# ivario123/r7020e-visual-odometry

Hardware: AMD Instinct MI355X
Metric: stereo frames/sec @1242x375 (SIFT detect+describe x2 + stereo matchFeatures) (higher is better)
Workload: dtype f32 (i8 MFMA for exact descriptor dot products); 1 GPU; BASELINE configs[1]: SIFT detect+describe + BF match on 1242x375 synthetic stereo, ~2k keypoints/image; rows=375, cols=1242, parallelism=frames sharded over 1 GPU(s)

## Files before the change

### r7020e-visual-odometry_amd/csrc/sift.hip

```cpp
#include "vo_internal.h"
#include <cstdlib>
#include <cstring>
#include <cmath>
#include <algorithm>
#include <utility>
#include <type_traits>
#include <mutex>

namespace vo {

struct Kern { float k[VO_SIFT_MAX_RADIUS + 1]; int r; float* nb; int nb_pitch, nb_rows, nb_cols; };

static int desc_radius_cap(const Pyramid& py, const vo_sift_params& p);

void build_pyramid_geometry(Pyramid& py, int rows, int cols, int n_img, const vo_sift_params& p)
{
    memset(&py, 0, sizeof(py));
    const int L = p.n_octave_layers;
    py.L = L;
    py.n_img = n_img;
    py.n_oct = vo_num_octaves(rows, cols, p.upsample);
    int R = p.upsample ? rows * 2 : rows, C = p.upsample ? cols * 2 : cols;
    size_t off = 0;
    size_t tmp_plane = 0;
// ... 1839 lines not shown
#ifndef VO_CPL2_MAXC
#define VO_CPL2_MAXC 1400
#endif
#ifndef VO_BLUR_MAX_TH
#define VO_BLUR_MAX_TH 128
#endif
#ifndef VO_BLUR_WAVES
#define VO_BLUR_WAVES 2048
#endif
        constexpr int kMaxTH = VO_BLUR_MAX_TH, kWaveTarget = VO_BLUR_WAVES, kCpl2MaxC = VO_CPL2_MAXC;
        const bool base = name[7] == 'b';
        const int cpl = (!base && C <= kCpl2MaxC) ? 2 : 4;
        const int n_strips = (C + 64 * cpl - 1) / (64 * cpl);
        const long rows_total = (long)R * n_strips * grid.z;
        int TH = (int)std::min<long>(base ? std::min(kMaxTH, kBaseMaxTH) : kMaxTH, rows_total / kWaveTarget);
        TH = std::max(BS_P, TH / BS_P * BS_P);
        if (R >= TH && R > RAD + BS_P + 2) {
            const int n_bands = (R + TH - 1) / TH;
#define VO_BS_GO(T, CP)                                                                                        \
    do {                                                                                                       \
        const int ns_ = (C + bs_sw(RAD, CP, T) - 1) / bs_sw(RAD, CP, T);                                       \
        VO_LAUNCH_NAMED(name, (k_blur_stream<RAD, T, CP>), dim3(ns_ * n_bands * (int)grid.z), dim3(64), 0, s, src, plane, \
                        dplane, pitch, R, C, g, K, ns_, n_bands, TH, isrc, in_rows, in_cols);                     \
    } while (0)
            if (base && src == nullptr) VO_BS_GO(5, 4);
            else if (base) VO_BS_GO(1, 4);
            else if (cpl == 2) VO_BS_GO(0, 2);
            else VO_BS_GO(0, 4);
#undef VO_BS_GO
            return true;
        }
    }
    if (lds > 64 * 1024) raise_lds_limit((const void*)k_blur_fused<RAD, MODE>);
    VO_LAUNCH_NAMED(MODE == 0 ? "k_blur_fused" : "k_blur_base", (k_blur_fused<RAD, MODE>), grid, dim3(256), lds, s, src,
                    plane, dplane, pitch, R, C, g, d, K, isrc, in_rows, in_cols);
    return false;
}

template <int MODE>
static bool launch_blur(dim3 grid, hipStream_t s, const float* src, size_t plane, size_t dplane, int pitch, int R, int C, float* g,
                        float* d, const Kern& K, const ImageSrc& isrc, int in_rows, int in_cols,
                        const char* name = MODE == 0 ? "k_blur_fused" : "k_blur_base")
{
    switch (K.r) {
    case 5: return launch_blur_r<5, MODE>(grid, s, src, plane, dplane, pitch, R, C, g, d, K, isrc, in_rows, in_cols, name);
    case 6: return launch_blur_r<6, MODE>(grid, s, src, plane, dplane, pitch, R, C, g, d, K, isrc, in_rows, in_cols, name);
    case 8: return launch_blur_r<8, MODE>(grid, s, src, plane, dplane, pitch, R, C, g, d, K, isrc, in_rows, in_cols, name);
    case 10: return launch_blur_r<10, MODE>(grid, s, src, plane, dplane, pitch, R, C, g, d, K, isrc, in_rows, in_cols, name);
    case 13: return launch_blur_r<13, MODE>(grid, s, src, plane, dplane, pitch, R, C, g, d, K, isrc, in_rows, in_cols, name);
    default: return launch_blur_r<0, MODE>(grid, s, src, plane, dplane, pitch, R, C, g, d, K, isrc, in_rows, in_cols, name);
    }
}

static float ext_threshold(const Pyramid& py, const vo_sift_params& p)
{
    return (float)floor(0.5 * p.contrast_threshold / py.L * 255.0);
}

struct SmallPlan { int o_small, rtab, cap, bcap; size_t lds; };
static SmallPlan small_plan(const Pyramid& py)
{
    SmallPlan sp{py.n_oct, 0, 0, 0, 0};
    int maxr = 0;
    for (int i = 1; i < py.L + 3; ++i) maxr = std::max(maxr, py.krad[i]);
    for (int o = py.n_oct - 1; o >= 1; --o) {
        int rt = 0, ct = 0, cap = 0, bcap = 0;
        bool fits = true;
        for (int q = o; q < py.n_oct; ++q) {
            fits = fits && py.oct[q].rows * py.oct[q].cols <= VO_SMALL_PX;
            cap = std::max(cap, py.oct[q].rows * py.oct[q].cols);
            if (q > o) bcap = std::max(bcap, py.oct[q].rows * py.oct[q].cols);
            rt = std::max(rt, py.oct[q].rows + 2 * maxr);
            ct = std::max(ct, py.oct[q].cols + 2 * maxr);
        }
        cap = (cap + 3) & ~3;
        bcap = (bcap + 3) & ~3;
        const size_t lds = sizeof(float) * (3 * (size_t)cap + bcap) + sizeof(int) * (rt + ct);
        if (!fits || lds > 160 * 1024) break;
        sp = SmallPlan{o, rt, cap, bcap, lds};
    }
    return sp;
}

int sift_small_octave(const Pyramid& py) { return small_plan(py).o_small; }

void sift_enqueue_small(const Pyramid& py, SiftBuffers& b, int n_img, hipStream_t s, const Pyramid* d_py)
{
    const SmallPlan sp = small_plan(py);
    if (sp.o_small >= py.n_oct) return;

    raise_lds_limit((const void*)k_small_pyr);
    VO_LAUNCH_NAMED("k_blur_small", k_small_pyr, dim3(n_img), dim3(VO_SMALL_T), sp.lds, s, d_py, b.arena, sp.o_small,
                    sp.rtab, sp.cap, sp.bcap);
}

void sift_enqueue_pyramid(const Pyramid& py, SiftBuffers& b, const ImageSrc& src, int n_img, const vo_sift_params& p,
                          hipStream_t s, const Pyramid* d_py, hipEvent_t ev_o0)
{
    const int L = py.L;
    float* A = b.arena;
    const SmallPlan sp = small_plan(py);
    const int o_small = sp.o_small;
    bool base_done = false;
    for (int o = 0; o < py.n_oct; ++o) {
        const OctGeom& g = py.oct[o];
        const int R = g.rows, C = g.cols;
        if (o == o_small) break;
        dim3 gf((C + FT_W - 1) / FT_W, (R + FT_H - 1) / FT_H, n_img);
        if (o == 0) {
            Kern K0 = make_kern(py, 0);
            const int rows = p.upsample ? R / 2 : R, cols = p.upsample ? C / 2 : C;
            const int r0 = K0.r;
            const bool stream_r = r0 == 5 || r0 == 6 || r0 == 8 || r0 == 10 || r0 == 13;
            if (p.upsample && stream_r && R >= 64) {
                launch_blur<0>(gf, s, nullptr, 0, py.istride, g.pitch, R, C, A + g.g_off[0], nullptr, K0, src, rows, cols,
                               "k_blur_base");
            } else {
                const dim3 qg((g.pitch / 4 + 255) / 256, R, n_img);
                if (p.upsample)
                    VO_LAUNCH(k_base_src<true>, qg, dim3(256), 0, s, src, rows, cols, b.tmp, g.plane, g.pitch, R, C, n_img);
                else
                    VO_LAUNCH(k_base_src<false>, qg, dim3(256), 0, s, src, rows, cols, b.tmp, g.plane, g.pitch, R, C, n_img);
                launch_blur<0>(gf, s, b.tmp, g.plane, py.istride, g.pitch, R, C, A + g.g_off[0], nullptr, K0, src, 0, 0,
                               "k_blur_base");
            }
        } else if (!base_done) {
            const OctGeom& pg = py.oct[o - 1];
            VO_LAUNCH(k_down, dim3((C + 255) / 256, R, n_img), dim3(256), 0, s, A + pg.g_off[L], py.istride, pg.pitch,
                      A + g.g_off[0], py.istride, g.pitch, C);
        }
        base_done = false;
        for (int i = 1; i < L + 3; ++i) {
            Kern K = make_kern(py, i);
            const bool emit = i == L && o + 1 < o_small;
            if (emit) {
                const OctGeom& ng = py.oct[o + 1];
                K.nb = A + ng.g_off[0];
                K.nb_pitch = ng.pitch; K.nb_rows = ng.rows; K.nb_cols = ng.cols;
            }
            const bool streamed = launch_blur<0>(gf, s, A + g.g_off[i - 1], py.istride, py.istride, g.pitch, R, C,
                                                 A + g.g_off[i], nullptr, K, src, 0, 0);
            if (emit) base_done = streamed;
        }
        if (o == 0 && ev_o0) hipEventRecord(ev_o0, s);
    }
}

#ifndef VO_FEATURE_GRID
#define VO_FEATURE_GRID 32768
#endif
constexpr int kFeatureGrid = VO_FEATURE_GRID;

void sift_enqueue_extrema(const Pyramid& py, SiftBuffers& b, int n_img, const vo_sift_params& p, hipStream_t s,
                          const Pyramid* d_py, int o_begin, int o_end)
{
    const int L = py.L;
    float* A = b.arena;
    const float thr = ext_threshold(py, p);
    const int u_first = py.ebase[o_begin], u_last = py.ebase[o_end];
    if (u_last > u_first) {
        const dim3 ge((u_last - u_first) * n_img);
#define VO_EXT_K(LL) VO_LAUNCH(k_ext_inner<LL>, ge, dim3(64), 0, s, d_py, A, b.mask, thr, n_img, u_first, u_last)
        switch (L) {
        case 1: VO_EXT_K(1); break;
        case 2: VO_EXT_K(2); break;
        case 3: VO_EXT_K(3); break;
        case 4: VO_EXT_K(4); break;
        default: VO_EXT_K(5); break;
        }
#undef VO_EXT_K
    }
}

void sift_enqueue_pyramid_tail(const Pyramid& py, SiftBuffers& b, int n_img, const vo_sift_params& p, hipStream_t s,
                               const Pyramid* d_py, int ext_o_begin)
{
    sift_enqueue_small(py, b, n_img, s, d_py);
    sift_enqueue_extrema(py, b, n_img, p, s, d_py, ext_o_begin, py.n_oct);
}

const char* sift_params_refusal(const vo_sift_params& p)
{
    if (p.n_octave_layers < 1 || p.n_octave_layers > 5) return "n_octave_layers";
    if (p.max_keypoints < 16) return "max_keypoints";
    if (!(p.sigma > 0.0f) || !std::isfinite(p.sigma)) return "sigma";
    if (!std::isfinite(p.contrast_threshold) || p.contrast_threshold < 0.0f) return "contrast_threshold";
    if (!std::isfinite(p.edge_threshold) || !(p.edge_threshold > 0.0f)) return "edge_threshold";
    const double scl = p.sigma * std::exp2((p.n_octave_layers + 0.5) / p.n_octave_layers);
    const double r = std::ceil(VO_SIFT_ORI_RADIUS * scl) + 1;
    const double per_column = std::floor(4294967296.0 / (361.0 * VO_DESC_FX_SCALE));
    if (!((2 * r + 1) * (2 * r + 1) <= VO_ORIENT_COLS * per_column)) return "sigma";
    if (!vo_sift_radii_ok(p.n_octave_layers, p.sigma, p.upsample)) return "sigma";
    return nullptr;
}

// ... 45 lines not shown
```

### r7020e-visual-odometry_amd/csrc/vo_api.hip

```cpp
#include "vo_internal.h"
#include "vo_geom.h"
#include <climits>
#include <cmath>
#include <cstdio>
#include <cstring>
#include <cstdarg>
#include <string>
#include <vector>
#include <deque>
#include <algorithm>

namespace vo {

Profiler* g_prof = nullptr;

void Profiler::begin(const char* name, hipStream_t s)
{
    if (used + 2 > (int)pool.size()) {
        int add = std::max(64, (int)pool.size());
        for (int i = 0; i < add; ++i) { hipEvent_t e; hipEventCreate(&e); pool.push_back(e); }
    }
    marks.push_back({name, used});
    hipEventRecord(pool[used], s);
    used += 1;
}

void Profiler::end(hipStream_t s)
{
    hipEventRecord(pool[used], s);
    used += 1;
}

void Profiler::collect()
{
    for (auto& m : marks) {
        float t = 0.0f;
        hipEventElapsedTime(&t, pool[m.second], pool[m.second + 1]);
        std::string n(m.first);
        size_t k = 0;
        for (; k < names.size(); ++k) if (names[k] == n) break;
        if (k == names.size()) { names.push_back(n); ms.push_back(0.0); calls.push_back(0); }
        ms[k] += t;
        calls[k] += 1;
    }
    marks.clear();
    used = 0;
}

void Profiler::reset_totals() { names.clear(); ms.clear(); calls.clear(); marks.clear(); used = 0; }

Profiler::~Profiler() { for (auto e : pool) hipEventDestroy(e); }

}

using namespace vo;

struct vo_ctx {
    int device = 0, rows = 0, cols = 0, max_batch = 0;
    vo_sift_params sp;
    vo_match_params mp;
    vo_ransac_params rp;
    vo_calib calib;
    bool has_calib = false;
    hipStream_t stream = nullptr;
    static constexpr int MAX_SUB = 4;
    int n_sub = 1;
    hipStream_t sub[MAX_SUB] = {};
    hipEvent_t ev_fork = nullptr, ev_join[MAX_SUB] = {}, ev_o0[MAX_SUB] = {};
    struct AuxSet {
        SiftBuffers sb;
        MatchBuffers mb;
        MatchJob* d_jobs = nullptr;
        int* pair_i = nullptr; int* pair_j = nullptr; int* pair_n = nullptr;
        GeomBuffers gb;
    } aux;
    hipEvent_t ev_done[2] = {};
    hipEvent_t ev_arena[2] = {};
    int next_set = 0, last_set = 0;
    Pyramid py;
    Pyramid* d_py = nullptr;
    SiftBuffers sb;
    MatchBuffers mb;
    MatchJob* d_jobs = nullptr;
    int* d_pair_i = nullptr;
    int* d_pair_j = nullptr;
    int* d_pair_n = nullptr;
    uint8_t* d_img = nullptr;
    uint8_t* d_cm = nullptr;
    size_t cm_cap = 0;
    bool ud_on[2] = {false, false};
    vo_bc_cam ud_cam[2] = {};
    uint8_t* d_rect = nullptr;
    int rect_B = 0;
    int strongest = 0;
    bool sel_used[2] = {false, false};
    uint8_t* d_fd[2] = {nullptr, nullptr};
    DescMeta* d_fm[2] = {nullptr, nullptr};
    int* d_fn = nullptr;
    float* d_ff[2] = {nullptr, nullptr};
    float* d_fa = nullptr;
    float* d_fbt = nullptr;
    int* d_fres = nullptr;
    MatchExBuffers mx;
    int* d_bad = nullptr;
    int* d_mi = nullptr; int* d_mj = nullptr; int* d_mn = nullptr;
    GeomBuffers gb;
    struct StepHost {
        FrameGeom* fg = nullptr; int* nkp = nullptr; int* ncand = nullptr; int* np = nullptr; int* rows = nullptr;
        int* ndet = nullptr;
        float* pX = nullptr; uint8_t* pkeep = nullptr;
        float* d_pX = nullptr; uint8_t* d_pkeep = nullptr;
        hipEvent_t ev = nullptr;
    };
    StepHost sh[VO_STEP_DEPTH];
    hipStream_t copy_stream = nullptr;
    struct Pending { int set, slot, B; bool first_tracked; bool sel; };
    std::deque<Pending> pending;
    int next_step_set = 0, next_slot = 0;
    std::vector<void*> lm_retired;
    int last_step_set = -1, last_step_B = 0;
    std::string err;
// ... 8 lines not shown
    uint8_t* d_lmkeep = nullptr;
    size_t lm_cap = 0, lm_n = 0;
    std::vector<long long> lm_frame_off{0};
    double* d_lmw_pose = nullptr;
    long long* d_lmw_off = nullptr;
    int lmw_cap = 0;
};

static std::string g_create_err;

static int fail(vo_ctx* c, int code, const char* fmt, ...)
{
    char buf[512];
    va_list ap;
    va_start(ap, fmt);
    vsnprintf(buf, sizeof(buf), fmt, ap);
    va_end(ap);
    if (c) c->err = buf; else g_create_err = buf;
    return code;
}

#define HIPC(c, x) do { hipError_t e_ = (x); if (e_ != hipSuccess) return fail(c, VO_ERR_HIP, "%s: %s (%s:%d)", #x, hipGetErrorString(e_), __FILE__, __LINE__); } while (0)

static const double I4[16] = {1, 0, 0, 0, 0, 1, 0, 0, 0, 0, 1, 0, 0, 0, 0, 1};

extern "C" {

void vo_default_sift_params(vo_sift_params* p)
{
    p->n_octave_layers = 3; p->sigma = 1.6f; p->contrast_threshold = 0.04f; p->edge_threshold = 10.0f;
    p->upsample = 1; p->max_keypoints = 16384;
}
void vo_default_match_params(vo_match_params* p) { p->match_threshold = 1.0f; p->max_ratio = 0.6f; }
void vo_default_match_opts(vo_match_opts* o) { o->match_threshold = 1.0f; o->max_ratio = 0.6f; o->unique = 0; o->reserved = 0; }
void vo_default_ransac_params(vo_ransac_params* p)
{
    p->max_num_trials = 1000; p->confidence = 99.0; p->max_reprojection_error = 1.0; p->seed = 0x5EED;
}

const char* vo_last_error(const vo_ctx* c) { return c ? c->err.c_str() : g_create_err.c_str(); }

void* vo_stream(vo_ctx* c) { return c ? (void*)c->stream : nullptr; }

static int job_stereo(const vo_ctx*, int f) { return f; }
static int job_track(const vo_ctx* c, int step, int f) { return c->max_batch + step * c->max_batch + f; }
static int job_single(const vo_ctx* c) { return 5 * c->max_batch; }

static void destroy_streams(vo_ctx* c)
{
    for (int k = 0; k < vo_ctx::MAX_SUB; ++k) {
        if (c->sub[k]) hipStreamDestroy(c->sub[k]);
        if (c->ev_join[k]) hipEventDestroy(c->ev_join[k]);
        if (c->ev_o0[k]) hipEventDestroy(c->ev_o0[k]);
        c->sub[k] = nullptr; c->ev_join[k] = nullptr; c->ev_o0[k] = nullptr;
    }
    if (c->ev_fork) hipEventDestroy(c->ev_fork);
    c->ev_fork = nullptr;
    for (int k = 0; k < 2; ++k) {
        if (c->ev_done[k]) hipEventDestroy(c->ev_done[k]);
        if (c->ev_arena[k]) hipEventDestroy(c->ev_arena[k]);
        c->ev_arena[k] = nullptr;
        c->ev_done[k] = nullptr;
    }
    for (int k = 0; k < VO_STEP_DEPTH; ++k) {
        if (c->sh[k].ev) hipEventDestroy(c->sh[k].ev);
        c->sh[k].ev = nullptr;
    }
    if (c->copy_stream) hipStreamDestroy(c->copy_stream);
    c->copy_stream = nullptr;
}

static void destroy_buffers(vo_ctx* c)
{
    sift_free(c->sb);
    match_free(c->mb);
    sift_free(c->aux.sb);
    match_free(c->aux.mb);
    hipFree(c->aux.d_jobs); hipFree(c->aux.pair_i); hipFree(c->aux.pair_j); hipFree(c->aux.pair_n);
    geom_free(c->aux.gb);
    for (int k = 0; k < VO_STEP_DEPTH; ++k) {
        hipHostFree(c->sh[k].fg); hipHostFree(c->sh[k].nkp); hipHostFree(c->sh[k].ncand); hipHostFree(c->sh[k].np); hipHostFree(c->sh[k].rows);
        hipHostFree(c->sh[k].ndet);
        hipHostFree(c->sh[k].pX); hipHostFree(c->sh[k].pkeep);
        hipFree(c->sh[k].d_pX); hipFree(c->sh[k].d_pkeep);
        const hipEvent_t ev = c->sh[k].ev;
        c->sh[k] = vo_ctx::StepHost();
        c->sh[k].ev = ev;
    }
    for (void* p : c->lm_retired) hipFree(p);
    c->lm_retired.clear();
    geom_free(c->gb);
    hipFree(c->d_py); hipFree(c->d_jobs); hipFree(c->d_pair_i); hipFree(c->d_pair_j); hipFree(c->d_pair_n);
    hipFree(c->d_rect);
    c->d_rect = nullptr;
    hipFree(c->d_img); hipFree(c->d_cm); hipFree(c->d_fd[0]); hipFree(c->d_fd[1]); hipFree(c->d_fm[0]); hipFree(c->d_fm[1]);
    hipFree(c->d_ff[0]); hipFree(c->d_ff[1]); hipFree(c->d_bad);
    hipFree(c->d_fa); hipFree(c->d_fbt); hipFree(c->d_fres);
    match_ex_free(c->mx);
    hipFree(c->d_fn); hipFree(c->d_mi); hipFree(c->d_mj); hipFree(c->d_mn);
    hipFree(c->d_lmX); hipFree(c->d_lmkeep); hipFree(c->d_lmw_pose); hipFree(c->d_lmw_off);
    c->d_lmX = nullptr; c->d_lmkeep = nullptr; c->d_lmw_pose = nullptr; c->d_lmw_off = nullptr;
    c->lm_cap = 0; c->lmw_cap = 0;
}

vo_ctx* vo_create(int device, int rows, int cols, int max_batch, const vo_calib* calib, const vo_sift_params* sift,
                  const vo_match_params* match, const vo_ransac_params* ransac)
{
    if (rows < 16 || cols < 16 || rows > 2048 || cols > 2048 || max_batch < 1 || max_batch > VO_MAX_BATCH) {
        fail(nullptr, VO_ERR_ARG, "vo_create: bad size rows=%d cols=%d max_batch=%d", rows, cols, max_batch);
        return nullptr;
    }
    {
        vo_sift_params sp;
        if (sift) sp = *sift; else vo_default_sift_params(&sp);
        if (const char* field = sift_params_refusal(sp)) {
            fail(nullptr, VO_ERR_ARG, "vo_create: unsupported sift params: %s (n_octave_layers=%d sigma=%g contrast_threshold=%g "
                 "edge_threshold=%g upsample=%d max_keypoints=%d)", field, sp.n_octave_layers, (double)sp.sigma,
                 (double)sp.contrast_threshold, (double)sp.edge_threshold, sp.upsample, sp.max_keypoints);
            return nullptr;
        }
    }
    if (hipSetDevice(device) != hipSuccess) { fail(nullptr, VO_ERR_HIP, "hipSetDevice(%d) failed", device); return nullptr; }
    vo_ctx* c = new vo_ctx();
    c->device = device; c->rows = rows; c->cols = cols; c->max_batch = max_batch;
    if (sift) c->sp = *sift; else vo_default_sift_params(&c->sp);
    if (match) c->mp = *match; else vo_default_match_params(&c->mp);
    if (ransac) c->rp = *ransac; else vo_default_ransac_params(&c->rp);
    if (calib) { c->calib = *calib; c->has_calib = true; }
    memcpy(c->pose, I4, sizeof(I4));
    auto bail = [&](const char* what, hipError_t e) -> vo_ctx* {
        fail(nullptr, VO_ERR_HIP, "vo_create: %s: %s", what, hipGetErrorString(e));
        destroy_buffers(c);
        destroy_streams(c);
        if (c->stream) hipStreamDestroy(c->stream);
        delete c;
        return nullptr;
    };
    hipError_t e;
    if ((e = hipStreamCreateWithFlags(&c->stream, hipStreamNonBlocking)) != hipSuccess) return bail("stream", e);
    for (int k = 0; k < vo_ctx::MAX_SUB; ++k) {
        e = hipStreamCreateWithFlags(&c->sub[k], hipStreamNonBlocking);
        if (e != hipSuccess) return bail("stream", e);
        if ((e = hipEventCreateWithFlags(&c->ev_join[k], hipEventDisableTiming)) != hipSuccess) return bail("event", e);
        if ((e = hipEventCreateWithFlags(&c->ev_o0[k], hipEventDisableTiming)) != hipSuccess) return bail("event", e);
    }
    if ((e = hipEventCreateWithFlags(&c->ev_fork, hipEventDisableTiming)) != hipSuccess) return bail("event", e);
    for (int k = 0; k < 2; ++k) {
        if ((e = hipEventCreateWithFlags(&c->ev_done[k], hipEventDisableTiming)) != hipSuccess) return bail("event", e);
        if ((e = hipEventCreateWithFlags(&c->ev_arena[k], hipEventDisableTiming)) != hipSuccess) return bail("event", e);
    }
    if ((e = hipStreamCreateWithFlags(&c->copy_stream, hipStreamNonBlocking)) != hipSuccess) return bail("stream", e);
    const int n_slots = 2 * max_batch + 2;
    const int kp_cap = c->sp.max_keypoints;
    build_pyramid_geometry(c->py, rows, cols, n_slots, c->sp);
    if ((e = hipMalloc((void**)&c->d_py, sizeof(Pyramid))) != hipSuccess) return bail("pyramid", e);
    if ((e = hipMemcpy(c->d_py, &c->py, sizeof(Pyramid), hipMemcpyHostToDevice)) != hipSuccess) return bail("pyramid copy", e);
    if ((e = sift_alloc(c->sb, c->py, kp_cap, 4 * kp_cap)) != hipSuccess) return bail("sift buffers", e);
    const int n_jobs = 5 * max_batch + 1;
    if ((e = match_alloc(c->mb, n_jobs, kp_cap)) != hipSuccess) return bail("match buffers", e);
    if ((e = hipMalloc((void**)&c->d_jobs, sizeof(MatchJob) * n_jobs)) != hipSuccess) return bail("jobs", e);
    const int pair_slots = max_batch + 1;
    if ((e = hipMalloc((void**)&c->d_pair_i, sizeof(int) * (size_t)pair_slots * kp_cap)) != hipSuccess) return bail("pairs", e);
    if ((e = hipMalloc((void**)&c->d_pair_j, sizeof(int) * (size_t)pair_slots * kp_cap)) != hipSuccess) return bail("pairs", e);
    if ((e = hipMalloc((void**)&c->d_pair_n, sizeof(int) * pair_slots)) != hipSuccess) return bail("pairs", e);
    if ((e = hipMemset(c->d_pair_n, 0, sizeof(int) * pair_slots)) != hipSuccess) return bail("pairs", e);
    if ((e = hipMalloc((void**)&c->d_img, (size_t)2 * max_batch * rows * cols)) != hipSuccess) return bail("staging", e);
    for (int k = 0; k < 2; ++k) {
        if ((e = hipMalloc((void**)&c->d_fd[k], (size_t)kp_cap * VO_DESC_LEN)) != hipSuccess) return bail("staging", e);
        if ((e = hipMalloc((void**)&c->d_fm[k], sizeof(DescMeta) * kp_cap)) != hipSuccess) return bail("staging", e);
        if ((e = hipMalloc((void**)&c->d_ff[k], sizeof(float) * kp_cap * VO_DESC_LEN)) != hipSuccess) return bail("staging", e);
    }
    if ((e = hipMalloc((void**)&c->d_fn, sizeof(int) * 2)) != hipSuccess) return bail("staging", e);
    if ((e = hipMalloc((void**)&c->d_bad, sizeof(int))) != hipSuccess) return bail("staging", e);
    if ((e = hipMalloc((void**)&c->d_mi, sizeof(int) * kp_cap)) != hipSuccess) return bail("staging", e);
    if ((e = hipMalloc((void**)&c->d_mj, sizeof(int) * kp_cap)) != hipSuccess) return bail("staging", e);
    if ((e = hipMalloc((void**)&c->d_mn, sizeof(int))) != hipSuccess) return bail("staging", e);
    if ((e = geom_alloc(c->gb, max_batch, kp_cap, c->rp.max_num_trials)) != hipSuccess) return bail("geometry buffers", e);
    std::vector<MatchJob> jobs(n_jobs);
    memset(jobs.data(), 0, sizeof(MatchJob) * n_jobs);
    const size_t dstride = (size_t)kp_cap * VO_DESC_LEN;
    for (int f = 0; f < max_batch; ++f) {
        MatchJob& J = jobs[job_stereo(c, f)];
        const int il = 2 * f, ir = 2 * f + 1;
        J.d1 = c->sb.desc + il * dstride; J.m1 = c->sb.meta + (size_t)il * kp_cap; J.idx1 = nullptr; J.n1 = c->sb.n_kp + il;
        J.d2 = c->sb.desc + ir * dstride; J.m2 = c->sb.meta + (size_t)ir * kp_cap; J.idx2 = nullptr; J.n2 = c->sb.n_kp + ir;
        J.out_i = c->d_pair_i + (size_t)f * kp_cap; J.out_j = c->d_pair_j + (size_t)f * kp_cap; J.out_n = c->d_pair_n + f;
        J.cap = kp_cap;
    }
    geom_fill_track_jobs(c->gb, jobs.data(), c->max_batch, job_track(c, 0, 0), c->sb, c->d_pair_i, c->d_pair_j, c->d_pair_n,
                         kp_cap);
    {
        MatchJob& J = jobs[job_single(c)];
        J.d1 = c->d_fd[0]; J.m1 = c->d_fm[0]; J.idx1 = nullptr; J.n1 = c->d_fn;
        J.d2 = c->d_fd[1]; J.m2 = c->d_fm[1]; J.idx2 = nullptr; J.n2 = c->d_fn + 1;
        J.out_i = c->d_mi; J.out_j = c->d_mj; J.out_n = c->d_mn; J.cap = kp_cap;
    }
    if ((e = hipMemcpy(c->d_jobs, jobs.data(), sizeof(MatchJob) * n_jobs, hipMemcpyHostToDevice)) != hipSuccess) return bail("jobs copy", e);
    {
// ... 46 lines not shown
    destroy_buffers(c);
    destroy_streams(c);
    if (c->stream) hipStreamDestroy(c->stream);
    delete c;
}

int vo_set_concurrency(vo_ctx* c, int n_streams)
{
    if (!c || n_streams < 1 || n_streams > vo_ctx::MAX_SUB) return VO_ERR_ARG;
    c->n_sub = n_streams;
    return VO_OK;
}

int vo_set_calib(vo_ctx* c, const vo_calib* calib)
{
    if (!c || !calib) return VO_ERR_ARG;
    c->calib = *calib;
    c->has_calib = true;
    return VO_OK;
}

int vo_set_profiling(vo_ctx* c, int enable)
{
    if (!c) return VO_ERR_ARG;
    c->prof.on = enable != 0;
    c->prof.reset_totals();
    return VO_OK;
}

static int finish(vo_ctx* c);
int vo_kernel_times(vo_ctx* c, const char** names, double* ms, int* calls, int capacity, int* n)
{
    if (!c) return VO_ERR_ARG;
    hipSetDevice(c->device);
    if (c->prof.on) {
        g_prof = &c->prof;
        int rc = finish(c);
        if (rc) return rc;
    }
    int m = (int)c->prof.names.size();
    if (n) *n = m;
    for (int i = 0; i < m && i < capacity; ++i) {
        if (names) names[i] = c->prof.names[i].c_str();
        if (ms) ms[i] = c->prof.ms[i];
        if (calls) calls[i] = c->prof.calls[i];
    }
    return VO_OK;
}

static int finish(vo_ctx* c)
{
    hipError_t e = hipStreamSynchronize(c->stream);
    for (int k = 0; k < 2 && e == hipSuccess; ++k) e = hipStreamSynchronize(c->sub[k]);
    if (e != hipSuccess) return fail(c, VO_ERR_HIP, "stream sync: %s", hipGetErrorString(e));
    e = hipGetLastError();
    if (e != hipSuccess) return fail(c, VO_ERR_HIP, "launch: %s", hipGetErrorString(e));
    if (c->prof.on) c->prof.collect();
    g_prof = nullptr;
    return VO_OK;
}
static int begin_call(vo_ctx* c, bool quiesce = true, bool step = false)
{
    hipSetDevice(c->device);
    if (!step && !c->pending.empty())
        return fail(c, VO_ERR_STATE, "asynchronous step batches pending (vo_step_collect first)");
    g_prof = c->prof.on ? &c->prof : nullptr;
    if (quiesce)
        for (int k = 0; k < 2; ++k) hipStreamWaitEvent(c->stream, c->ev_done[k], 0);
    return VO_OK;
}
#define BEGIN_CALL(...) do { int rc_ = begin_call(__VA_ARGS__); if (rc_) return rc_; } while (0)

__global__ __launch_bounds__(256) void k_cm_to_rm_u8(const uint8_t* __restrict__ src, int ld, int rows, int cols,
                                                     uint8_t* __restrict__ dst)
{
    __shared__ uint8_t t[32][33];
    const int n = blockIdx.z, r0 = blockIdx.x * 32, c0 = blockIdx.y * 32;
    const uint8_t* s = src + (size_t)n * ld * cols;
    uint8_t* d = dst + (size_t)n * rows * cols;
    const int tx = threadIdx.x & 31, ty = threadIdx.x >> 5;
    for (int k = ty; k < 32; k += 8) {
        const int c = c0 + k, r = r0 + tx;
        if (c < cols && r < rows) t[k][tx] = s[(size_t)c * ld + r];
    }
    __syncthreads();
    for (int k = ty; k < 32; k += 8) {
        const int r = r0 + k, c = c0 + tx;
        if (r < rows && c < cols) d[(size_t)r * cols + c] = t[tx][k];
    }
}

static int stage_images(vo_ctx* c, const uint8_t* img, int ld, int col_major, int n, uint8_t* dst)
{
    const int rows = c->rows, cols = c->cols;
    if (!col_major) {
        HIPC(c, hipMemcpy2DAsync(dst, cols, img, ld, cols, (size_t)rows * n, hipMemcpyHostToDevice, c->stream));
        return VO_OK;
    }
    const size_t need = (size_t)ld * ((size_t)cols * n - 1) + rows;
    if (need > c->cm_cap) {
        HIPC(c, hipStreamSynchronize(c->stream));
        hipFree(c->d_cm);
        c->d_cm = nullptr;
        c->cm_cap = 0;
        HIPC(c, hipMalloc((void**)&c->d_cm, need));
        c->cm_cap = need;
// ... 355 lines not shown
    if (!bad) {
        BEGIN_CALL(c);
        return match_staged_ex(c, n1, n2, p, unique, pairs, metric, capacity, n_pairs, "vo_match_f32_ex");
    }
    if ((rc = f32_buffers(c, "vo_match_f32_ex")) != VO_OK || (rc = match_ex_buffers(c, "vo_match_f32_ex")) != VO_OK) return rc;
    BEGIN_CALL(c);
    match_f32_launch_ex(c->d_ff[0], n1, ld1, c->d_ff[1], n2, ld2, col_major, c->d_fa, c->d_fbt, c->d_fres, c->mx.metric,
                        c->mx.back, p, unique, c->stream);
    std::vector<int> res((size_t)n1 + 1), back((size_t)n2 + 1);
    std::vector<float> best((size_t)n1 + 1);
    if (n1) HIPC(c, hipMemcpyAsync(res.data(), c->d_fres, sizeof(int) * n1, hipMemcpyDeviceToHost, c->stream));
    if (n1) HIPC(c, hipMemcpyAsync(best.data(), c->mx.metric, sizeof(float) * n1, hipMemcpyDeviceToHost, c->stream));
    if (unique && n1 && n2) HIPC(c, hipMemcpyAsync(back.data(), c->mx.back, sizeof(int) * n2, hipMemcpyDeviceToHost, c->stream));
    rc = finish(c);
    if (rc) return rc;
    int P = 0;
    for (int i = 0; i < n1; ++i) {
        if (res[i] < 0 || (unique && back[res[i]] != i)) continue;
        if (P < capacity) {
            if (pairs) { pairs[2 * P] = (uint32_t)i + 1; pairs[2 * P + 1] = (uint32_t)res[i] + 1; }
            if (metric) metric[P] = best[i];
        }
        ++P;
    }
    if (n_pairs) *n_pairs = P;
    if (P > capacity) return fail(c, VO_ERR_CAPACITY, "vo_match_f32_ex: %d pairs exceed capacity %d", P, capacity);
    return VO_OK;
}

static int capacity_flags(const SiftBuffers& sb, const int* nkp, const int* ncand, int n)
{
    int fl = 0;
    for (int i = 0; i < n; ++i) {
        if (nkp[i] > sb.kp_cap) fl |= VO_FLAG_KEYPOINTS;
        if (ncand[i] > sb.cand_cap) fl |= VO_FLAG_CANDIDATES;
    }
    return fl;
}

struct SetRef {
    SiftBuffers* sb; MatchBuffers* mb; MatchJob* jobs; int* pair_i; int* pair_j; int* pair_n;
    GeomBuffers* gb; MatchJob* track_jobs;
};
static SetRef set_ref(vo_ctx* c, int set)
{
    if (set == 0)
        return {&c->sb, &c->mb, c->d_jobs + job_stereo(c, 0), c->d_pair_i, c->d_pair_j, c->d_pair_n, &c->gb,
                c->d_jobs + job_track(c, 0, 0)};
    return {&c->aux.sb, &c->aux.mb, c->aux.d_jobs, c->aux.pair_i, c->aux.pair_j, c->aux.pair_n, &c->aux.gb,
            c->aux.d_jobs + job_track(c, 0, 0)};
}

static int enqueue_sift_stereo(vo_ctx* c, int set, const uint8_t* d_l, const uint8_t* d_r, int B, bool join,
                               bool fork = true)
{
    const size_t fs = (size_t)c->rows * c->cols;
    const int parts = std::min(c->n_sub, B);
    SetRef S = set_ref(c, set);
    hipStream_t sp = c->sub[0], st = c->sub[1];
    if (fork) {
        HIPC(c, hipEventRecord(c->ev_fork, c->stream));
        HIPC(c, hipStreamWaitEvent(sp, c->ev_fork, 0));
    }
    HIPC(c, hipStreamWaitEvent(sp, c->ev_arena[set], 0));
    const int o_small = sift_small_octave(c->py);
    const bool undist = c->ud_on[0] || c->ud_on[1];
    if (undist) c->rect_B = B;
    c->sel_used[set] = c->strongest > 0;
    for (int p = 0; p < parts; ++p) {
        const int f0 = B * p / parts, nf = B * (p + 1) / parts - f0;
        const uint8_t* pl = d_l + f0 * fs;
        const uint8_t* pr = d_r + f0 * fs;
        if (undist) {
            UndistortSide U[2];
            for (int k = 0; k < 2; ++k) {
                U[k].cam = c->ud_cam[k];
                U[k].in = k ? pr : pl;
                U[k].out = c->d_rect + ((size_t)k * c->max_batch + f0) * fs;
                U[k].copy = c->ud_on[k] ? 0 : 1;
                U[k].pad = 0;
            }
            undistort_launch(U, 2, c->rows, c->cols, nf, fs, fs, sp);
            pl = U[0].out;
            pr = U[1].out;
        }
        ImageSrc src{pl, pr, fs, c->cols, 0};
        SiftBuffers v = sift_view(*S.sb, c->py, 2 * f0, 2 * nf);
        sift_enqueue_pyramid(c->py, v, src, 2 * nf, c->sp, sp, c->d_py, c->ev_o0[p]);
        sift_enqueue_small(c->py, v, 2 * nf, sp, c->d_py);
        HIPC(c, hipEventRecord(c->ev_join[p], sp));
    }
    for (int p = 0; p < parts; ++p) {
        const int f0 = B * p / parts, nf = B * (p + 1) / parts - f0;
        SiftBuffers v = sift_view(*S.sb, c->py, 2 * f0, 2 * nf);
        const bool iso = c->prof.on && join;
        HIPC(c, hipStreamWaitEvent(st, iso ? c->ev_join[p] : c->ev_o0[p], 0));
        sift_enqueue_extrema(c->py, v, 2 * nf, c->sp, st, c->d_py, 0, 1);
        HIPC(c, hipStreamWaitEvent(st, c->ev_join[p], 0));
        sift_enqueue_extrema(c->py, v, 2 * nf, c->sp, st, c->d_py, 1, o_small);
        sift_enqueue_extrema(c->py, v, 2 * nf, c->sp, st, c->d_py, o_small, c->py.n_oct);
        sift_enqueue_features(c->py, v, 2 * nf, c->sp, st, c->d_py, c->strongest);
        if (p == parts - 1) HIPC(c, hipEventRecord(c->ev_arena[set], st));
        match_launch(match_view(*S.mb, f0), S.jobs + f0, nf, c->mp, st);
    }
    HIPC(c, hipEventRecord(c->ev_done[set], st));
    if (join) HIPC(c, hipStreamWaitEvent(c->stream, c->ev_done[set], 0));
    c->last_set = set;
    return VO_OK;
}

int vo_sift_match_batch_dev(vo_ctx* c, const uint8_t* d_lefts, const uint8_t* d_rights, int B, vo_pair_stats* stats)
{
    if (!c || !d_lefts || !d_rights || B < 1 || B > c->max_batch) return fail(c, VO_ERR_ARG, "vo_sift_match_batch_dev: bad arguments");
    BEGIN_CALL(c, false);
    const int set = c->next_set;
    c->next_set ^= 1;
    const bool sync = stats != nullptr;
    int rc = enqueue_sift_stereo(c, set, d_lefts, d_rights, B, sync);
    if (rc) return rc;
    c->last_B = B;
    if (!sync) {
        g_prof = nullptr;
        hipError_t e = hipGetLastError();
        if (e != hipSuccess) return fail(c, VO_ERR_HIP, "launch: %s", hipGetErrorString(e));
        return VO_OK;
    }
    SetRef S = set_ref(c, set);
    std::vector<int> nk(2 * B), nc(2 * B), np(B);
    std::vector<int> nd;
    HIPC(c, hipMemcpyAsync(nk.data(), S.sb->n_kp, sizeof(int) * 2 * B, hipMemcpyDeviceToHost, c->stream));
    if (c->strongest > 0) {
        nd.resize(2 * B);
        HIPC(c, hipMemcpyAsync(nd.data(), S.sb->n_det, sizeof(int) * 2 * B, hipMemcpyDeviceToHost, c->stream));
    }
    HIPC(c, hipMemcpyAsync(nc.data(), S.sb->n_cand, sizeof(int) * 2 * B, hipMemcpyDeviceToHost, c->stream));
    HIPC(c, hipMemcpyAsync(np.data(), S.pair_n, sizeof(int) * B, hipMemcpyDeviceToHost, c->stream));
    rc = finish(c);
    if (rc) return rc;
    if (stats) {
        for (int f = 0; f < B; ++f) {
            stats[f].n_left = nk[2 * f]; stats[f].n_right = nk[2 * f + 1]; stats[f].n_stereo = np[f];
            stats[f].flags = capacity_flags(c->sb, (nd.empty() ? nk : nd).data() + 2 * f, nc.data() + 2 * f, 2);
        }
    }
    return VO_OK;
}

int vo_fetch_keypoints(vo_ctx* c, int image, vo_keypoint* kps, uint8_t* desc, int capacity, int* n)
{
    if (!c || image < 0 || image >= c->sb.n_img) return fail(c, VO_ERR_ARG, "vo_fetch_keypoints: bad image");
    hipSetDevice(c->device);
    HIPC(c, hipStreamSynchronize(c->stream));
    HIPC(c, hipEventSynchronize(c->ev_done[c->last_set]));
    const SiftBuffers& B = (c->last_set == 1 && image < 2 * c->max_batch) ? c->aux.sb : c->sb;
    int cnt = 0;
    HIPC(c, hipMemcpy(&cnt, B.n_kp + image, sizeof(int), hipMemcpyDeviceToHost));
    if (n) *n = cnt;
    int m = std::min(std::min(cnt, B.kp_cap), capacity);
    if (m > 0) {
        if (kps) HIPC(c, hipMemcpy(kps, B.kp + (size_t)image * B.kp_cap, sizeof(vo_keypoint) * m, hipMemcpyDeviceToHost));
        if (desc) HIPC(c, hipMemcpy(desc, B.desc + (size_t)image * B.kp_cap * VO_DESC_LEN, (size_t)m * VO_DESC_LEN, hipMemcpyDeviceToHost));
    }
    return VO_OK;
}

int vo_fetch_candidate_counts(vo_ctx* c, int image, int* n_cand, int* n_accepted)
{
    if (!c || image < 0 || image >= c->sb.n_img) return fail(c, VO_ERR_ARG, "vo_fetch_candidate_counts: bad image");
    hipSetDevice(c->device);
    HIPC(c, hipStreamSynchronize(c->stream));
    HIPC(c, hipEventSynchronize(c->ev_done[c->last_set]));
// ... 71 lines not shown
    a.rp = c->rp;
    return a;
}

static void mat4_mul(const double* A, const double* B, double* C)
{
    double T[16];
    for (int i = 0; i < 4; ++i)
        for (int j = 0; j < 4; ++j)
            T[4 * i + j] = A[4 * i] * B[j] + A[4 * i + 1] * B[4 + j] + A[4 * i + 2] * B[8 + j] + A[4 * i + 3] * B[12 + j];
    memcpy(C, T, sizeof(T));
}

static void lm_world(const double* pose, const float* X, double* out)
{
    const double x0 = X[0], x1 = X[1], x2 = X[2];
    for (int a = 0; a < 3; ++a) {
        double w = pose[4 * a] * x0 + pose[4 * a + 1] * x1 + pose[4 * a + 2] * x2 + pose[4 * a + 3];
        out[a] = (double)(float)w;
    }
}

static int enqueue_carry(vo_ctx* c, int from, int f, int to)
{
    const int M = c->max_batch, K = c->sb.kp_cap;
    SetRef A = set_ref(c, from), Z = set_ref(c, to);
    for (int side = 0; side < 2; ++side) {
        const int src = 2 * f + side, dst = 2 * M + side;
        HIPC(c, hipMemcpyAsync(Z.sb->kp + (size_t)dst * K, A.sb->kp + (size_t)src * K, sizeof(vo_keypoint) * K,
                               hipMemcpyDeviceToDevice, c->stream));
        HIPC(c, hipMemcpyAsync(Z.sb->desc + (size_t)dst * K * VO_DESC_LEN, A.sb->desc + (size_t)src * K * VO_DESC_LEN,
                               (size_t)K * VO_DESC_LEN, hipMemcpyDeviceToDevice, c->stream));
        HIPC(c, hipMemcpyAsync(Z.sb->meta + (size_t)dst * K, A.sb->meta + (size_t)src * K, sizeof(DescMeta) * K,
                               hipMemcpyDeviceToDevice, c->stream));
        HIPC(c, hipMemcpyAsync(Z.sb->n_kp + dst, A.sb->n_kp + src, sizeof(int), hipMemcpyDeviceToDevice, c->stream));
        if (c->strongest > 0)
            HIPC(c, hipMemcpyAsync(Z.sb->n_det + dst, A.sb->n_det + src, sizeof(int), hipMemcpyDeviceToDevice, c->stream));
    }
    HIPC(c, hipMemcpyAsync(Z.pair_i + (size_t)M * K, A.pair_i + (size_t)f * K, sizeof(int) * K, hipMemcpyDeviceToDevice, c->stream));
    HIPC(c, hipMemcpyAsync(Z.pair_j + (size_t)M * K, A.pair_j + (size_t)f * K, sizeof(int) * K, hipMemcpyDeviceToDevice, c->stream));
    HIPC(c, hipMemcpyAsync(Z.pair_n + M, A.pair_n + f, sizeof(int), hipMemcpyDeviceToDevice, c->stream));
    return VO_OK;
}

static int submit_batch(vo_ctx* c, const uint8_t* d_l, const uint8_t* d_r, int B, bool fork)
{
    if (!c->has_calib) return fail(c, VO_ERR_STATE, "vo_step: no calibration (vo_set_calib)");
    if (c->pending.size() >= VO_STEP_DEPTH)
        return fail(c, VO_ERR_STATE, "vo_step_submit_dev: %d batches already pending (collect first)", VO_STEP_DEPTH);
    const int set = c->next_step_set, slot = c->next_slot;
    SetRef S = set_ref(c, set);
    for (const vo_ctx::Pending& q : c->pending)
        if (q.set == set) HIPC(c, hipStreamWaitEvent(c->sub[1], c->sh[q.slot].ev, 0));
    int rc = enqueue_sift_stereo(c, set, d_l, d_r, B, true, fork);
    if (rc) return rc;
    StepArgs a = step_args(c, B, set);
    geom_enqueue(*S.gb, *S.mb, S.track_jobs, a, c->mp, c->stream);
    vo_ctx::StepHost& H = c->sh[slot];
    HIPC(c, hipMemcpyAsync(H.fg, S.gb->fg, sizeof(FrameGeom) * B, hipMemcpyDeviceToHost, c->stream));
    HIPC(c, hipMemcpyAsync(H.nkp, S.sb->n_kp, sizeof(int) * 2 * B, hipMemcpyDeviceToHost, c->stream));
    if (c->strongest > 0)
        HIPC(c, hipMemcpyAsync(H.ndet, S.sb->n_det, sizeof(int) * 2 * B, hipMemcpyDeviceToHost, c->stream));
    HIPC(c, hipMemcpyAsync(H.ncand, S.sb->n_cand, sizeof(int) * 2 * B, hipMemcpyDeviceToHost, c->stream));
    HIPC(c, hipMemcpyAsync(H.np, S.pair_n, sizeof(int) * B, hipMemcpyDeviceToHost, c->stream));
    HIPC(c, hipMemcpyAsync(H.rows, S.gb->lm_rows, sizeof(int) * B, hipMemcpyDeviceToHost, c->stream));
    lm_pack_launch(*S.gb, B, H.d_pX, H.d_pkeep, c->stream);
    if ((rc = enqueue_carry(c, set, B - 1, set ^ 1))) return rc;
    HIPC(c, hipEventRecord(H.ev, c->stream));
    hipError_t e = hipGetLastError();
    if (e != hipSuccess) return fail(c, VO_ERR_HIP, "launch: %s", hipGetErrorString(e));
    c->pending.push_back({set, slot, B, c->have_features, c->strongest > 0});
    c->next_step_set ^= 1;
    c->next_slot = (slot + 1) % VO_STEP_DEPTH;
    c->have_features = true;
    c->frame_index += B;
    return VO_OK;
}

static int collect_batch(vo_ctx* c, vo_step_out* outs, int capacity, int* n_out)
{
    if (c->pending.empty()) return fail(c, VO_ERR_STATE, "vo_step_collect: no batch pending");
    const vo_ctx::Pending P = c->pending.front();
    if (capacity < P.B) return fail(c, VO_ERR_CAPACITY, "vo_step_collect: %d frames pending, capacity %d", P.B, capacity);
    const int K = c->sb.kp_cap, B = P.B;
    const vo_ctx::StepHost& H = c->sh[P.slot];
    if (c->prof.on) {
        g_prof = &c->prof;
        int rc = finish(c);
        if (rc) return rc;
    } else {
        HIPC(c, hipEventSynchronize(H.ev));
    }
    size_t total = 0;
    std::vector<size_t> roff(B + 1, 0);
    for (int f = 0; f < B; ++f) roff[f + 1] = roff[f] + (size_t)std::min(H.rows[f], K);
    total = roff[B];
    if (c->lm_camera) {
        const size_t first = (P.first_tracked ? 0 : roff[1]), add = total - first;
        if (add > 0) {
            if (c->lm_n + add > c->lm_cap) {
                size_t cap = std::max<size_t>({c->lm_n + add, 2 * c->lm_cap, (size_t)1 << 16});
                float* nX = nullptr; uint8_t* nk = nullptr;
                if (hipMalloc((void**)&nX, sizeof(float) * 3 * cap) != hipSuccess ||
                    hipMalloc((void**)&nk, cap) != hipSuccess) {
                    hipFree(nX);
                    return fail(c, VO_ERR_HIP, "vo_step_collect: landmark store of %zu rows", cap);
                }
// ... 229 lines not shown
    HIPC(c, hipMemcpyAsync(c->d_lmw_pose, poses, sizeof(double) * 16 * nf, hipMemcpyHostToDevice, c->stream));
    HIPC(c, hipMemcpyAsync(c->d_lmw_off, c->lm_frame_off.data(), sizeof(long long) * (nf + 1), hipMemcpyHostToDevice,
                           c->stream));
    lm_world_launch(c->d_lmw_pose, c->d_lmw_off, nf, c->d_lmX, c->d_lmkeep, d_out, c->stream);
    hipError_t e = hipGetLastError();
    if (e != hipSuccess) return fail(c, VO_ERR_HIP, "launch: %s", hipGetErrorString(e));
    HIPC(c, hipStreamSynchronize(c->stream));
    return VO_OK;
}

int vo_landmarks_to_world(const double pose[16], const float* X, const uint8_t* keep, int n, double* out)
{
    if (!pose || n < 0 || (n > 0 && (!X || !keep || !out))) return VO_ERR_ARG;
    for (int m = 0; m < n; ++m) {
        if (keep[m]) lm_world(pose, X + (size_t)m * 3, out + (size_t)m * 3);
        else out[3 * m] = out[3 * m + 1] = out[3 * m + 2] = 0.0;
    }
    return VO_OK;
}

int vo_chain_poses(const double* rel, const int32_t* status, int n, const double* pose0, double* out)
{
    if (n < 0 || (n > 0 && (!rel || !out))) return VO_ERR_ARG;
    double pose[16];
    memcpy(pose, pose0 ? pose0 : I4, sizeof(pose));
    for (int f = 0; f < n; ++f) {
        if (!status || status[f] == VO_OK) mat4_mul(pose, rel + (size_t)16 * f, pose);
        memcpy(out + (size_t)16 * f, pose, sizeof(pose));
    }
    return VO_OK;
}

int vo_landmarks_to_world_frames(const double* poses, const int32_t* rows_per_frame, int n_frames, const float* X,
                                 const uint8_t* keep, long n_rows, double* out)
{
    if (n_frames < 0 || n_rows < 0 || (n_frames > 0 && (!poses || !rows_per_frame))) return VO_ERR_ARG;
    long r = 0;
    for (int f = 0; f < n_frames; ++f) {
        const long k = rows_per_frame[f];
        if (k < 0 || r + k > n_rows) return VO_ERR_ARG;
        int rc = vo_landmarks_to_world(poses + (size_t)16 * f, X + 3 * r, keep + r, (int)k, out + 3 * r);
        if (rc) return rc;
        r += k;
    }
    return r == n_rows ? VO_OK : VO_ERR_ARG;
}

int vo_reset(vo_ctx* c)
{
    if (!c) return VO_ERR_ARG;
    hipSetDevice(c->device);
    HIPC(c, hipStreamSynchronize(c->stream));
    for (int k = 0; k < vo_ctx::MAX_SUB; ++k) HIPC(c, hipStreamSynchronize(c->sub[k]));
    HIPC(c, hipStreamSynchronize(c->copy_stream));
    c->pending.clear();
    c->next_step_set = 0;
    c->next_slot = 0;
    for (void* p : c->lm_retired) hipFree(p);
    c->lm_retired.clear();
    c->last_step_set = -1;
    c->have_features = false;
    c->frame_index = 0;
    memcpy(c->pose, I4, sizeof(I4));
    c->landmarks.clear();
    c->lm_n = 0;
    c->lm_frame_off.assign(1, 0);
    HIPC(c, hipMemset(c->d_pair_n + c->max_batch, 0, sizeof(int)));
    HIPC(c, hipMemset(c->aux.pair_n + c->max_batch, 0, sizeof(int)));
    return VO_OK;
}

int vo_set_frame_index(vo_ctx* c, long frame_index)
{
    if (!c || frame_index < 0) return VO_ERR_ARG;
    c->frame_index = frame_index;
    return VO_OK;
}

static int upload_desc(vo_ctx* c, int slot, const uint8_t* d, int n)
{
    const int K = c->sb.kp_cap;
    if (n) HIPC(c, hipMemcpyAsync(c->sb.desc + (size_t)slot * K * VO_DESC_LEN, d, (size_t)n * VO_DESC_LEN, hipMemcpyHostToDevice, c->stream));
    desc_meta_launch(c->sb.desc + (size_t)slot * K * VO_DESC_LEN, c->sb.meta + (size_t)slot * K, n, c->stream);
    HIPC(c, hipMemcpyAsync(c->sb.n_kp + slot, &n, sizeof(int), hipMemcpyHostToDevice, c->stream));
    HIPC(c, hipStreamSynchronize(c->stream));
    return VO_OK;
}

int vo_track(vo_ctx* c, const uint8_t* old_l, const uint8_t* old_r, int n_old, const uint8_t* cur_l, int n_cl,
             const uint8_t* cur_r, int n_cr, uint32_t* idx_out, int capacity, int* K_out)
{
    if (!c || n_old < 0 || n_cl < 0 || n_cr < 0) return fail(c, VO_ERR_ARG, "vo_track: bad arguments");
    const int K = c->sb.kp_cap, M = c->max_batch;
    if (n_old > K || n_cl > K || n_cr > K) return fail(c, VO_ERR_CAPACITY, "vo_track: more rows than max_keypoints");
    BEGIN_CALL(c);
    c->have_features = false;
    c->last_set = 0;
    c->sel_used[0] = false;
    int rc;
    if ((rc = upload_desc(c, 2 * M, old_l, n_old))) return rc;
    if ((rc = upload_desc(c, 2 * M + 1, old_r, n_old))) return rc;
    if ((rc = upload_desc(c, 0, cur_l, n_cl))) return rc;
    if ((rc = upload_desc(c, 1, cur_r, n_cr))) return rc;
    std::vector<int> iota(std::max(n_old, 1));
    for (int k = 0; k < n_old; ++k) iota[k] = k;
    if (n_old) {
// ... 131 lines not shown
```

### r7020e-visual-odometry_amd/csrc/vo_internal.h

```cpp
#pragma once
#include <hip/hip_runtime.h>
#include <stdint.h>
#include <vector>
#include <string>
#include "vo.h"
#include "vo_spec.h"

#define VO_WAVE 64

namespace vo {

struct Profiler {
    bool on = false;
    std::vector<hipEvent_t> pool;
    int used = 0;
    std::vector<std::pair<const char*, int>> marks;
    std::vector<std::string> names;
    std::vector<double> ms;
    std::vector<int> calls;
    void begin(const char* name, hipStream_t s);
    void end(hipStream_t s);
    void collect();
    void reset_totals();
    ~Profiler();
// ... 54 lines not shown
    int o, layer, r, c;
    int npk, pad0, pad1, pad2;
    float ang[VO_SIFT_MAX_PEAKS + 2];
};

struct KpInt {
    float xo, yo, scl, angle;
    int o, layer, pad0, pad1;
};

struct DescMeta {
    int32_t sum;
    float inv_norm;
};

struct SiftBuffers {
    float* arena = nullptr;
    float* tmp = nullptr;
    unsigned long long* mask = nullptr;
    uint32_t* woff = nullptr;
    uint32_t* cand = nullptr;
    int* n_cand = nullptr;
    int* acc = nullptr;
    int* n_acc = nullptr;
    CandOut* cout = nullptr;
    uint32_t* koff = nullptr;
    int* n_kp = nullptr;
    int* n_det = nullptr;
    unsigned long long* skey = nullptr;
    uint32_t* snpk = nullptr;
    vo_keypoint* kp = nullptr;
    KpInt* kpi = nullptr;
    uint8_t* desc = nullptr;
    DescMeta* meta = nullptr;
    int cand_cap = 0, kp_cap = 0, n_img = 0;
};

struct ImageSrc {
    const uint8_t* left;
    const uint8_t* right;
    size_t frame_stride;
    int ld;
    int pad;
};

void build_pyramid_geometry(Pyramid& py, int rows, int cols, int n_img, const vo_sift_params& p);
const char* sift_params_refusal(const vo_sift_params& p);
SiftBuffers sift_view(const SiftBuffers& b, const Pyramid& py, int img0, int n);
hipError_t sift_alloc(SiftBuffers& b, const Pyramid& py, int kp_cap, int cand_cap);
hipError_t sift_alloc_select(SiftBuffers& b);
void sift_free(SiftBuffers& b);
void sift_enqueue(const Pyramid& py, SiftBuffers& b, const ImageSrc& src, int n_img,
                  const vo_sift_params& p, hipStream_t s, const Pyramid* d_py, int strongest = 0);
void sift_enqueue_pyramid(const Pyramid& py, SiftBuffers& b, const ImageSrc& src, int n_img,
                          const vo_sift_params& p, hipStream_t s, const Pyramid* d_py, hipEvent_t ev_o0 = nullptr);
void sift_enqueue_pyramid_tail(const Pyramid& py, SiftBuffers& b, int n_img, const vo_sift_params& p, hipStream_t s,
                               const Pyramid* d_py, int ext_o_begin);
void sift_enqueue_extrema(const Pyramid& py, SiftBuffers& b, int n_img, const vo_sift_params& p, hipStream_t s,
                          const Pyramid* d_py, int o_begin, int o_end);
int sift_small_octave(const Pyramid& py);
void sift_enqueue_small(const Pyramid& py, SiftBuffers& b, int n_img, hipStream_t s, const Pyramid* d_py);
void sift_enqueue_features(const Pyramid& py, SiftBuffers& b, int n_img, const vo_sift_params& p, hipStream_t s,
                           const Pyramid* d_py, int strongest = 0);

#define VO_UD_CHUNK 16
struct UndistortSide {
    vo_bc_cam cam;
    const uint8_t* in;
    uint8_t* out;
    int copy, pad;
};
void undistort_launch(const UndistortSide* sides, int n_sides, int rows, int cols, int B, size_t in_stride,
                      size_t out_stride, hipStream_t s);

#if VO_EXPERIMENTAL
extern int g_exp_msac_eager;
#endif
void raise_lds_limit(const void* fn);

struct MatchJob {
    const uint8_t* d1; const DescMeta* m1; const int* idx1; const int* n1;
    const uint8_t* d2; const DescMeta* m2; const int* idx2; const int* n2;
    int* out_i;
    int* out_j;
    int* out_n;
    int cap;
    int pad;
};

struct MatchTop2 { float best; int idx; float second; int pad; };

struct MatchBuffers {
    MatchJob* jobs = nullptr;
    MatchTop2* partial = nullptr;
    int max_jobs = 0, row_cap = 0, n_chunks = 0;
};

#ifndef VO_MATCH_CHUNK
#define VO_MATCH_CHUNK 4096
#endif

hipError_t match_alloc(MatchBuffers& b, int max_jobs, int row_cap);
MatchBuffers match_view(const MatchBuffers& b, int k0);
void match_free(MatchBuffers& b);
struct MatchCompose {
    int* lists; int* list_n;
    const int* pair_i; const int* pair_j;
    int M, kp_cap, step;
// ... 25 lines not shown
```

Baseline: 10050 stereo frames/s.

## Fork lower pyramid octaves onto a separate stream to overlap with upper octaves

```diff
diff --git a/r7020e-visual-odometry_amd/csrc/sift.hip b/r7020e-visual-odometry_amd/csrc/sift.hip
--- a/r7020e-visual-odometry_amd/csrc/sift.hip
+++ b/r7020e-visual-odometry_amd/csrc/sift.hip
@@ -1915,6 +1915,13 @@
     }
 }
 
+static bool blur_latency_bound(int R, int C, int n_img)
+{
+    const int cpl = C <= VO_CPL2_MAXC ? 2 : 4;
+    const long n_strips = (C + 64 * cpl - 1) / (64 * cpl);
+    return (long)R * n_strips * n_img / VO_BLUR_WAVES < VO_BLUR_MAX_TH;
+}
+
 static float ext_threshold(const Pyramid& py, const vo_sift_params& p)
 {
     return (float)floor(0.5 * p.contrast_threshold / py.L * 255.0);
@@ -1958,17 +1965,21 @@
 }
 
 void sift_enqueue_pyramid(const Pyramid& py, SiftBuffers& b, const ImageSrc& src, int n_img, const vo_sift_params& p,
-                          hipStream_t s, const Pyramid* d_py, hipEvent_t ev_o0)
+                          hipStream_t s, const Pyramid* d_py, hipEvent_t ev_o0, const ScaleChains& ch)
 {
     const int L = py.L;
     float* A = b.arena;
     const SmallPlan sp = small_plan(py);
     const int o_small = sp.o_small;
+    const bool forked = ch.down != nullptr && ch.down != s;
+    int o_fork = std::min(1, o_small - 1);
+    while (o_fork + 1 < o_small && !blur_latency_bound(py.oct[o_fork + 1].rows, py.oct[o_fork + 1].cols, n_img)) ++o_fork;
     bool base_done = false;
     for (int o = 0; o < py.n_oct; ++o) {
         const OctGeom& g = py.oct[o];
         const int R = g.rows, C = g.cols;
         if (o == o_small) break;
+        if (forked && o == o_fork + 1) s = ch.down;
         dim3 gf((C + FT_W - 1) / FT_W, (R + FT_H - 1) / FT_H, n_img);
         if (o == 0) {
             Kern K0 = make_kern(py, 0);
@@ -2004,6 +2015,10 @@
             const bool streamed = launch_blur<0>(gf, s, A + g.g_off[i - 1], py.istride, py.istride, g.pitch, R, C,
                                                  A + g.g_off[i], nullptr, K, src, 0, 0);
             if (emit) base_done = streamed;
+            if (forked && o == o_fork && i == L) {
+                hipEventRecord(ch.ev_fork, s);
+                hipStreamWaitEvent(ch.down, ch.ev_fork, 0);
+            }
         }
         if (o == 0 && ev_o0) hipEventRecord(ev_o0, s);
     }
diff --git a/r7020e-visual-odometry_amd/csrc/vo_api.hip b/r7020e-visual-odometry_amd/csrc/vo_api.hip
--- a/r7020e-visual-odometry_amd/csrc/vo_api.hip
+++ b/r7020e-visual-odometry_amd/csrc/vo_api.hip
@@ -67,6 +67,8 @@
     int n_sub = 1;
     hipStream_t sub[MAX_SUB] = {};
     hipEvent_t ev_fork = nullptr, ev_join[MAX_SUB] = {}, ev_o0[MAX_SUB] = {};
+    hipStream_t down = nullptr;
+    hipEvent_t ev_down[MAX_SUB] = {}, ev_top[MAX_SUB] = {};
     struct AuxSet {
         SiftBuffers sb;
         MatchBuffers mb;
@@ -181,8 +183,12 @@
         if (c->sub[k]) hipStreamDestroy(c->sub[k]);
         if (c->ev_join[k]) hipEventDestroy(c->ev_join[k]);
         if (c->ev_o0[k]) hipEventDestroy(c->ev_o0[k]);
-        c->sub[k] = nullptr; c->ev_join[k] = nullptr; c->ev_o0[k] = nullptr;
-    }
+        if (c->ev_down[k]) hipEventDestroy(c->ev_down[k]);
+        if (c->ev_top[k]) hipEventDestroy(c->ev_top[k]);
+        c->sub[k] = nullptr; c->ev_join[k] = nullptr; c->ev_o0[k] = nullptr; c->ev_down[k] = nullptr; c->ev_top[k] = nullptr;
+    }
+    if (c->down) hipStreamDestroy(c->down);
+    c->down = nullptr;
     if (c->ev_fork) hipEventDestroy(c->ev_fork);
     c->ev_fork = nullptr;
     for (int k = 0; k < 2; ++k) {
@@ -272,7 +278,10 @@
         if (e != hipSuccess) return bail("stream", e);
         if ((e = hipEventCreateWithFlags(&c->ev_join[k], hipEventDisableTiming)) != hipSuccess) return bail("event", e);
         if ((e = hipEventCreateWithFlags(&c->ev_o0[k], hipEventDisableTiming)) != hipSuccess) return bail("event", e);
-    }
+        if ((e = hipEventCreateWithFlags(&c->ev_down[k], hipEventDisableTiming)) != hipSuccess) return bail("event", e);
+        if ((e = hipEventCreateWithFlags(&c->ev_top[k], hipEventDisableTiming)) != hipSuccess) return bail("event", e);
+    }
+    if ((e = hipStreamCreateWithFlags(&c->down, hipStreamNonBlocking)) != hipSuccess) return bail("stream", e);
     if ((e = hipEventCreateWithFlags(&c->ev_fork, hipEventDisableTiming)) != hipSuccess) return bail("event", e);
     for (int k = 0; k < 2; ++k) {
         if ((e = hipEventCreateWithFlags(&c->ev_done[k], hipEventDisableTiming)) != hipSuccess) return bail("event", e);
@@ -425,6 +434,7 @@
 {
     hipError_t e = hipStreamSynchronize(c->stream);
     for (int k = 0; k < 2 && e == hipSuccess; ++k) e = hipStreamSynchronize(c->sub[k]);
+    if (e == hipSuccess) e = hipStreamSynchronize(c->down);
     if (e != hipSuccess) return fail(c, VO_ERR_HIP, "stream sync: %s", hipGetErrorString(e));
     e = hipGetLastError();
     if (e != hipSuccess) return fail(c, VO_ERR_HIP, "launch: %s", hipGetErrorString(e));
@@ -886,12 +896,14 @@
 }
 
 static int enqueue_sift_stereo(vo_ctx* c, int set, const uint8_t* d_l, const uint8_t* d_r, int B, bool join,
-                               bool fork = true)
+                               bool chains, bool fork = true)
 {
     const size_t fs = (size_t)c->rows * c->cols;
     const int parts = std::min(c->n_sub, B);
     SetRef S = set_ref(c, set);
     hipStream_t sp = c->sub[0], st = c->sub[1];
+    const bool iso = c->prof.on && join;
+    const hipStream_t sd = (iso || !chains) ? sp : c->down;
     if (fork) {
         HIPC(c, hipEventRecord(c->ev_fork, c->stream));
         HIPC(c, hipStreamWaitEvent(sp, c->ev_fork, 0));
@@ -920,16 +932,20 @@
         }
         ImageSrc src{pl, pr, fs, c->cols, 0};
         SiftBuffers v = sift_view(*S.sb, c->py, 2 * f0, 2 * nf);
-        sift_enqueue_pyramid(c->py, v, src, 2 * nf, c->sp, sp, c->d_py, c->ev_o0[p]);
-        sift_enqueue_small(c->py, v, 2 * nf, sp, c->d_py);
-        HIPC(c, hipEventRecord(c->ev_join[p], sp));
+        ScaleChains ch;
+        ch.down = sd;
+        ch.ev_fork = c->ev_down[p];
+        sift_enqueue_pyramid(c->py, v, src, 2 * nf, c->sp, sp, c->d_py, c->ev_o0[p], ch);
+        HIPC(c, hipEventRecord(c->ev_top[p], sp));
+        sift_enqueue_small(c->py, v, 2 * nf, sd, c->d_py);
+        HIPC(c, hipEventRecord(c->ev_join[p], sd));
     }
     for (int p = 0; p < parts; ++p) {
         const int f0 = B * p / parts, nf = B * (p + 1) / parts - f0;
         SiftBuffers v = sift_view(*S.sb, c->py, 2 * f0, 2 * nf);
-        const bool iso = c->prof.on && join;
         HIPC(c, hipStreamWaitEvent(st, iso ? c->ev_join[p] : c->ev_o0[p], 0));
         sift_enqueue_extrema(c->py, v, 2 * nf, c->sp, st, c->d_py, 0, 1);
+        HIPC(c, hipStreamWaitEvent(st, c->ev_top[p], 0));
         HIPC(c, hipStreamWaitEvent(st, c->ev_join[p], 0));
         sift_enqueue_extrema(c->py, v, 2 * nf, c->sp, st, c->d_py, 1, o_small);
         sift_enqueue_extrema(c->py, v, 2 * nf, c->sp, st, c->d_py, o_small, c->py.n_oct);
@@ -950,7 +966,7 @@
     const int set = c->next_set;
     c->next_set ^= 1;
     const bool sync = stats != nullptr;
-    int rc = enqueue_sift_stereo(c, set, d_lefts, d_rights, B, sync);
+    int rc = enqueue_sift_stereo(c, set, d_lefts, d_rights, B, sync, true);
     if (rc) return rc;
     c->last_B = B;
     if (!sync) {
@@ -1128,7 +1144,7 @@
     SetRef S = set_ref(c, set);
     for (const vo_ctx::Pending& q : c->pending)
         if (q.set == set) HIPC(c, hipStreamWaitEvent(c->sub[1], c->sh[q.slot].ev, 0));
-    int rc = enqueue_sift_stereo(c, set, d_l, d_r, B, true, fork);
+    int rc = enqueue_sift_stereo(c, set, d_l, d_r, B, true, false, fork);
     if (rc) return rc;
     StepArgs a = step_args(c, B, set);
     geom_enqueue(*S.gb, *S.mb, S.track_jobs, a, c->mp, c->stream);
@@ -1464,6 +1480,7 @@
     hipSetDevice(c->device);
     HIPC(c, hipStreamSynchronize(c->stream));
     for (int k = 0; k < vo_ctx::MAX_SUB; ++k) HIPC(c, hipStreamSynchronize(c->sub[k]));
+    HIPC(c, hipStreamSynchronize(c->down));
     HIPC(c, hipStreamSynchronize(c->copy_stream));
     c->pending.clear();
     c->next_step_set = 0;
diff --git a/r7020e-visual-odometry_amd/csrc/vo_internal.h b/r7020e-visual-odometry_amd/csrc/vo_internal.h
--- a/r7020e-visual-odometry_amd/csrc/vo_internal.h
+++ b/r7020e-visual-odometry_amd/csrc/vo_internal.h
@@ -130,8 +130,13 @@
 void sift_free(SiftBuffers& b);
 void sift_enqueue(const Pyramid& py, SiftBuffers& b, const ImageSrc& src, int n_img,
                   const vo_sift_params& p, hipStream_t s, const Pyramid* d_py, int strongest = 0);
+struct ScaleChains {
+    hipStream_t down = nullptr;
+    hipEvent_t ev_fork = nullptr;
+};
 void sift_enqueue_pyramid(const Pyramid& py, SiftBuffers& b, const ImageSrc& src, int n_img,
-                          const vo_sift_params& p, hipStream_t s, const Pyramid* d_py, hipEvent_t ev_o0 = nullptr);
+                          const vo_sift_params& p, hipStream_t s, const Pyramid* d_py, hipEvent_t ev_o0 = nullptr,
+                          const ScaleChains& ch = ScaleChains());
 void sift_enqueue_pyramid_tail(const Pyramid& py, SiftBuffers& b, int n_img, const vo_sift_params& p, hipStream_t s,
                                const Pyramid* d_py, int ext_o_begin);
 void sift_enqueue_extrema(const Pyramid& py, SiftBuffers& b, int n_img, const vo_sift_params& p, hipStream_t s,
```

New measurement: 10230 stereo frames/s (median of 6 runs). +1.8%, better.
